# sterngerlach/my-lidar-graph-slam-v2

Hardware: AMD Instinct MI355X
Metric: candidate poses scored/sec (CSM+BnB), 1/2/4/8 GPU; % HBM roofline (higher is better)
Workload: dtype f32+u32; 1 GPU; configs[1]: frontend CSM, 1080-beam scan, 400x400@5cm grid, +-2 m/+-30 deg window at 5 cm/0.5 deg, L=4; distinct_scans=512, mode=csm_score_windows_dev, 256 windows per launch chain, 12 chains per step, beams=1080, parallelism=single GPU, poses_found=3072

## Files before the change

### include/csm_hip.h

```cpp
#ifndef CSM_HIP_H
#define CSM_HIP_H

#include <stdint.h>

#ifdef __cplusplus
extern "C" {
#endif

#define CSM_OK       0
#define CSM_ENOENT  (-2)
#define CSM_EIO     (-5)
#define CSM_ENOMEM  (-12)
#define CSM_ENODEV  (-19)
#define CSM_EINVAL  (-22)

#define CSM_FLAG_EDGE_BAND   1u
#define CSM_FLAG_KEY_TIE     2u
#define CSM_FLAG_F64_TIE     4u
#define CSM_FLAG_LITERAL     8u
#define CSM_FLAG_PROJ_DELTA 16u

typedef struct csm_ctx csm_ctx;

#define CSM_TUNE_NO_LANE_MAP         1u
#define CSM_TUNE_NO_XCD_MAP          2u
#define CSM_TUNE_NO_PAIR_TAIL        4u
#define CSM_TUNE_NO_TWO_SLICES       8u
#define CSM_TUNE_NO_THETA_MAJOR     16u
#define CSM_TUNE_NO_TILE_SPLIT      32u
#define CSM_TUNE_MAP_HOST_PROJECTION 64u
#define CSM_TUNE_NO_JOINT          128u
#define CSM_TUNE_NO_BOUND_PASS     256u
#define CSM_TUNE_NO_TWO_PHASE      512u
#define CSM_TUNE_FORCE_TWO_PHASE  1024u
#define CSM_TUNE_NO_GRAPHS        2048u

typedef struct {
    int32_t  device_id;
    uint32_t tuning_off;
    int32_t  map_uncertain_cap;
    int32_t  reserved[5];
} csm_config;

typedef struct {
    double  resolution;
    double  offset_x;
    double  offset_y;
} csm_geometry;

typedef struct {
// ... 114 lines not shown
int  csm_score_windows_dump_dev(csm_ctx* ctx, int32_t n, const uint64_t* map_ids,
                                const csm_window* windows, const int32_t* const* hit_col_dev,
                                const int32_t* const* hit_row_dev, csm_result* out_dev,
                                uint32_t* const* dump_s_dev, uint16_t* const* dump_k_dev,
                                float* const* dump_f_dev);
typedef struct {
    int64_t nominal_candidates;
    int64_t coarse_nodes_scored;
    int64_t fine_candidates_scored;
    int32_t two_phase;
    int32_t graph_replayed;
    int64_t blocks_scored, blocks_skipped;
} csm_search_info;
int  csm_last_search_info(csm_ctx* ctx, csm_search_info* out);
int  csm_bound_pass_stats(csm_ctx* ctx, uint64_t* blocks_scored, uint64_t* blocks_skipped);
int  csm_resolve_window_dev(csm_ctx* ctx, uint64_t map_id, const csm_window* w,
                            const int32_t* hit_col_dev, const int32_t* hit_row_dev,
                            csm_result* out_dev);
int  csm_score_window_dump(csm_ctx* ctx, uint64_t map_id, const csm_window* w,
                           const int32_t* hit_col, const int32_t* hit_row,
                           csm_result* out, uint32_t* dump_s, uint16_t* dump_k,
                           uint16_t* dump_coarse_k);

int  csm_correlative_match(csm_ctx* ctx, uint64_t map_id,
                           const csm_geometry* geom, const csm_scan* scan,
                           const double initial_pose[3],
                           const csm_correlative_params* params,
                           csm_summary* out);

int  csm_bnb_match_batch(csm_ctx* ctx, const csm_loop_query* queries,
// ... 515 lines not shown
                     const double* query_travel, int32_t n_q, const csm_loop_search_params* params,
                     csm_loop_candidate* out, int32_t* counts, csm_loop_search_info* info);
int  csm_host_loop_candidates_nearest(const csm_loop_candidate* cands, const int32_t* counts, int32_t n_q,
                                      int32_t n_per_query, int32_t n_total, csm_loop_candidate* out,
                                      int32_t* n_out);

int  csm_enable_kernel_timing(csm_ctx* ctx, int32_t enable);
int  csm_kernel_time(csm_ctx* ctx, const char* name, double* total_ms,
                     int64_t* launches);
int  csm_reset_kernel_timing(csm_ctx* ctx);

const char* csm_version(void);

int  csm_debug_live_bytes(int64_t* device, int64_t* pinned);
int  csm_debug_grid_known(csm_ctx* ctx, uint64_t map_id, int32_t out[2]);

#ifdef __cplusplus
}
#endif
#endif
```

### my-lidar-graph-slam-v2_amd/csm_hip/_lib.py

```python
import ctypes as C
import importlib.util
import os
import sys

_HERE = os.path.dirname(os.path.abspath(__file__))
LIB_PATH = os.environ.get("CSM_HIP_LIB") or os.path.join(os.path.dirname(_HERE), "csrc", "libcsm_hip.so")

CSM_OK = 0
CSM_ENOENT = -2
CSM_EIO = -5
CSM_ENOMEM = -12
CSM_ENODEV = -19
CSM_EINVAL = -22

FLAG_EDGE_BAND = 1
FLAG_KEY_TIE = 2
FLAG_F64_TIE = 4
FLAG_LITERAL = 8
FLAG_PROJ_DELTA = 16


class Config(C.Structure):
    _fields_ = [("device_id", C.c_int32), ("tuning_off", C.c_uint32), ("map_uncertain_cap", C.c_int32),
                ("reserved", C.c_int32 * 5)]


TUNE_NO_LANE_MAP, TUNE_NO_XCD_MAP, TUNE_NO_PAIR_TAIL, TUNE_NO_TWO_SLICES = 1, 2, 4, 8
TUNE_NO_THETA_MAJOR, TUNE_NO_TILE_SPLIT, TUNE_MAP_HOST_PROJECTION, TUNE_NO_JOINT = 16, 32, 64, 128
TUNE_NO_BOUND_PASS = 256
TUNE_NO_TWO_PHASE, TUNE_FORCE_TWO_PHASE, TUNE_NO_GRAPHS = 512, 1024, 2048
TUNE_GREEDY_LITERAL_SUMS = 4096
GREEDY_KERNEL_SIZE_MAX = 8
GROUP_FORCE_RCCL = 1


class SearchInfo(C.Structure):
    _fields_ = [("nominal_candidates", C.c_int64), ("coarse_nodes_scored", C.c_int64),
                ("fine_candidates_scored", C.c_int64), ("two_phase", C.c_int32), ("graph_replayed", C.c_int32),
                ("blocks_scored", C.c_int64), ("blocks_skipped", C.c_int64)]


class Geometry(C.Structure):
    _fields_ = [("resolution", C.c_double), ("offset_x", C.c_double),
                ("offset_y", C.c_double)]


# ... 312 lines not shown
                                   C.c_void_p, C.c_void_p, C.c_int32, C.c_void_p,
                                   C.c_void_p, C.c_void_p, C.c_void_p]),
    "csm_host_probability_lut": (None, [C.c_void_p]),
    "csm_project_scan": (C.c_int, [_ctx, _P(Geometry), C.c_void_p, C.c_double, C.c_int32, C.c_void_p,
                                   C.c_void_p, C.c_int32, C.c_void_p, C.c_void_p, C.c_void_p, C.c_int32,
                                   _P(C.c_int32)]),
    "csm_score_window": (C.c_int, [_ctx, C.c_uint64, _P(Window), C.c_void_p,
                                   C.c_void_p, _P(Result)]),
    "csm_score_window_dev": (C.c_int, [_ctx, C.c_uint64, _P(Window), C.c_void_p,
                                       C.c_void_p, C.c_void_p]),
    "csm_score_windows_dev": (C.c_int, [_ctx, C.c_int32, C.c_void_p, C.c_void_p, C.c_void_p, C.c_void_p,
                                        C.c_void_p]),
    "csm_score_windows_dump_dev": (C.c_int, [_ctx, C.c_int32, C.c_void_p, C.c_void_p, C.c_void_p, C.c_void_p,
                                             C.c_void_p, C.c_void_p, C.c_void_p, C.c_void_p]),
    "csm_bound_pass_stats": (C.c_int, [_ctx, _P(C.c_uint64), _P(C.c_uint64)]),
    "csm_last_search_info": (C.c_int, [_ctx, C.c_void_p]),
    "csm_resolve_window_dev": (C.c_int, [_ctx, C.c_uint64, _P(Window), C.c_void_p,
                                         C.c_void_p, C.c_void_p]),
    "csm_score_window_dump": (C.c_int, [_ctx, C.c_uint64, _P(Window), C.c_void_p,
                                        C.c_void_p, _P(Result), C.c_void_p,
                                        C.c_void_p, C.c_void_p]),
    "csm_correlative_match": (C.c_int, [_ctx, C.c_uint64, _P(Geometry), _P(Scan),
                                        C.c_void_p, _P(CorrelativeParams), _P(Summary)]),
    "csm_score_window_peaks": (C.c_int, [_ctx, C.c_uint64, _P(Window), C.c_void_p, C.c_void_p, _P(PeaksParams),
                                         _P(Result), _P(C.c_int32)]),
    "csm_correlative_peaks": (C.c_int, [_ctx, C.c_uint64, _P(Geometry), _P(Scan), C.c_void_p,
                                        _P(CorrelativeParams), _P(PeaksParams), _P(Summary), _P(C.c_int32)]),
    "csm_correlative_peaks_batch": (C.c_int, [_ctx, _P(LoopQuery), C.c_int32, _P(CorrelativeParams),
                                              _P(PeaksParams), _P(Summary), _P(C.c_int32)]),
    "csm_score_window_moments": (C.c_int, [_ctx, C.c_uint64, _P(Window), C.c_void_p, C.c_void_p, _P(VolumeParams),
# ... 95 lines not shown
    "csm_group_size": (C.c_int32, [C.c_void_p]),
    "csm_group_member": (C.c_void_p, [C.c_void_p, C.c_int32]),
    "csm_group_last_error": (C.c_char_p, [C.c_void_p]),
    "csm_group_bnb_match_batch": (C.c_int, [C.c_void_p, _P(LoopQuery), C.c_int32, _P(BnbParams), _P(Summary)]),
    "csm_group_correlative_match_batch": (C.c_int, [C.c_void_p, _P(LoopQuery), C.c_int32,
                                                    _P(CorrelativeParams), _P(Summary)]),
    "csm_allgather_results": (C.c_int, [C.c_void_p, C.c_void_p]),
    "csm_group_gathered_records_dev": (C.c_int, [C.c_void_p, C.c_int32, _P(C.c_void_p), _P(C.c_int32)]),
    "csm_group_exchange_info": (C.c_int, [C.c_void_p, _P(C.c_int32), _P(C.c_double)]),
    "csm_enable_kernel_timing": (C.c_int, [_ctx, C.c_int32]),
    "csm_kernel_time": (C.c_int, [_ctx, C.c_char_p, _P(C.c_double), _P(C.c_int64)]),
    "csm_reset_kernel_timing": (C.c_int, [_ctx]),
    "csm_version": (C.c_char_p, []),
    "csm_debug_live_bytes": (C.c_int, [_P(C.c_int64), _P(C.c_int64)]),
    "csm_debug_grid_known": (C.c_int, [_ctx, C.c_uint64, _P(C.c_int32)]),
}

_lib = None


def load():
    global _lib
    if _lib is not None:
        return _lib
    if not os.path.exists(LIB_PATH):
        raise ImportError(
            "libcsm_hip.so not built: run `python -c 'import __graft_entry__ as g; g.build()'` "
            "(expected at %s)" % LIB_PATH)
    if "torch" not in sys.modules and importlib.util.find_spec("torch") is not None:
        import torch
# ... 8 lines not shown
```

### my-lidar-graph-slam-v2_amd/csm_hip/api.py

```python
import contextlib
import ctypes as C

import numpy as np

from . import _lib as L


class CsmError(RuntimeError):
    def __init__(self, code, text):
        super().__init__("csm_hip error %d: %s" % (code, text))
        self.code = code


def _ptr(a):
    return a.ctypes.data_as(C.c_void_p)


def _f64(a):
    return np.ascontiguousarray(a, dtype=np.float64)


def _scan_nodes(nodes, as_f64, keep):
    arr = (L.ScanNode * max(len(nodes), 1))()
    for i, nd in enumerate(nodes):
# ... 691 lines not shown
            raise ValueError("upload_grid_blocks: every block must be (%d, %d)" % (side, side))
        ptrs = (C.c_void_p * len(keep))(*[None if b is None else b.ctypes.data for b in keep])
        self._check(self.lib.csm_upload_grid_blocks(self._ctx, map_id, ptrs, block_rows, block_cols, log2_block))
        self.shapes[map_id] = (block_rows << log2_block, block_cols << log2_block)

    def has_grid(self, map_id):
        return bool(self.lib.csm_has_grid(self._ctx, map_id))

    def debug_grid_known(self, map_id):
        out = (C.c_int32 * 2)()
        rc = self.lib.csm_debug_grid_known(self._ctx, map_id, out)
        if rc != 0:
            raise CsmError(rc, "csm_debug_grid_known: map %d not resident" % map_id)
        return out[0], out[1]

    def release_grid(self, map_id):
        self._check(self.lib.csm_release_grid(self._ctx, map_id))
        self.shapes.pop(map_id, None)

    def build_pyramid(self, map_id, win_sizes):
        w = np.ascontiguousarray(win_sizes, dtype=np.int32)
        self._check(self.lib.csm_build_pyramid(
            self._ctx, map_id, w.ctypes.data_as(C.POINTER(C.c_int32)), w.size))

    def project_scan(self, geom, sensor_pose, step_theta, win_theta, angles, ranges, cap=1 << 20):
        a, r = _f64(angles), _f64(ranges)
        n, nt = a.size, 2 * win_theta + 1
        col = np.zeros((nt, n), np.int32)
        row = np.zeros((nt, n), np.int32)
        unc = np.zeros(cap, np.uint32)
# ... 86 lines not shown
        n, ids, wins, cols, rows = prepared

        def arr(ptrs):
            return (C.c_void_p * n)(*[p or None for p in ptrs]) if ptrs is not None else None
        self._check(self.lib.csm_score_windows_dump_dev(self._ctx, n, ids, wins, cols, rows, C.c_void_p(out_ptr),
                                                        arr(dump_s_ptrs), arr(dump_k_ptrs), arr(dump_f_ptrs)))

    def last_search_info(self):
        info = L.SearchInfo()
        self._check(self.lib.csm_last_search_info(self._ctx, C.byref(info)))
        return {k: getattr(info, k) for k, _ in info._fields_}

    def bound_pass_stats(self):
        a, b = C.c_uint64(0), C.c_uint64(0)
        self._check(self.lib.csm_bound_pass_stats(self._ctx, C.byref(a), C.byref(b)))
        return a.value, b.value

    def correlative_match(self, map_id, geom, angles, ranges, rel_pose, init_pose,
                          range_x, range_y, range_theta, low_resolution,
                          score_threshold=0.0, known_rate_threshold=0.0):
        scan, keep = _scan_struct(angles, ranges, rel_pose)
        g = L.Geometry(*geom)
        p = _correlative_params(range_x, range_y, range_theta, low_resolution, score_threshold, known_rate_threshold)
        init = _f64(init_pose)
        out = L.Summary()
        self._check(self.lib.csm_correlative_match(self._ctx, map_id, C.byref(g), C.byref(scan),
                                                   _ptr(init), C.byref(p), C.byref(out)))
        return summary_to_dict(out)

    @staticmethod
# ... 671 lines not shown
```

### my-lidar-graph-slam-v2_amd/csrc/csm_api.hip

```cpp
#include "csm_matchers.hpp"
#include "csm_certify.hpp"

namespace csm_host {

void base_changed(DeviceGrid& g)
{
    g.phase.clear();
    ++g.base_epoch;
}

void free_levels(DeviceGrid& g, bool keep_base)
{
    base_changed(g);
    if (!keep_base) {
        g.xg.reset();
        g.xgf.reset();
        g.alloc.reset();
        g.xg_stale = true;
        g.xgf_valid = false;
        g.alloc_log2 = kDefaultLog2Block;
        g.alloc_derived = true;
        g.alloc_stale = true;
    }
    g.levels.resize(keep_base && !g.levels.empty() ? 1 : 0);
// ... 38 lines not shown
        return CSM_ENODEV;
    const int dev = cfg ? cfg->device_id : 0;
    if (dev < 0 || dev >= ndev)
        return CSM_ENODEV;
    csm_ctx* ctx = new csm_ctx();
    ctx->device = dev;
    {
        Tuning& t = ctx->tune;
        const uint32_t off = cfg ? cfg->tuning_off : 0u;
        t.lane_map = !(off & CSM_TUNE_NO_LANE_MAP);
        t.xcd_map = !(off & CSM_TUNE_NO_XCD_MAP);
        t.pair_tail = !(off & CSM_TUNE_NO_PAIR_TAIL);
        t.two_slices = !(off & CSM_TUNE_NO_TWO_SLICES);
        t.joint = !(off & CSM_TUNE_NO_JOINT);
        t.bound_pass = !(off & CSM_TUNE_NO_BOUND_PASS);
        t.two_phase = (off & CSM_TUNE_NO_TWO_PHASE) ? -1 : (off & CSM_TUNE_FORCE_TWO_PHASE) ? 1 : 0;
        t.graphs = !(off & CSM_TUNE_NO_GRAPHS);
        t.tile_split = !(off & CSM_TUNE_NO_TILE_SPLIT);
        t.map_host_projection = (off & CSM_TUNE_MAP_HOST_PROJECTION) != 0;
        t.greedy_literal = (off & CSM_TUNE_GREEDY_LITERAL_SUMS) != 0;
        if (off & CSM_TUNE_NO_THETA_MAJOR)
            t.theta_major = 0;
        t.map_unc_cap = cfg ? cfg->map_uncertain_cap : 0;
#ifdef CSM_TUNING
        auto env_int = [](const char* name, int dflt) {
            const char* e = getenv(name);
            return e ? atoi(e) : dflt;
        };
        t.lane_map = env_int("CSM_LANE_MAP", t.lane_map) != 0;
        t.xcd_map = env_int("CSM_XCD_MAP", t.xcd_map) != 0;
// ... 454 lines not shown
```

### my-lidar-graph-slam-v2_amd/csrc/csm_batch.hip

```cpp
#include "csm_matchers.hpp"

#include <optional>

#ifdef CSM_BIN_TIMING
static unsigned long long* g_bin_debug = nullptr;
static uint32_t* bin_debug_buffer()
{
    const size_t bytes = (size_t)kBinDebugRows * 128;
    if (!g_bin_debug && (hipMalloc(reinterpret_cast<void**>(&g_bin_debug), bytes) != hipSuccess ||
                         hipMemset(g_bin_debug, 0, bytes) != hipSuccess))
        g_bin_debug = nullptr;
    return reinterpret_cast<uint32_t*>(g_bin_debug);
}
#endif

namespace csm_host {


struct BatchPrep : WindowFrame {
    DeviceGrid* grid = nullptr;
    int level[kMaxElig] = { 0 };
    int n_theta = 0, n = 0;
    int win_x = 0, win_y = 0, win_t = 0;
    int max_tiles = 0;
// ... 420 lines not shown
    F = score_job(gr, gr.levels[p.level[0]].cells, 1, B, min_known);
    F.joint = joint ? 1 : 0;
    F.rank_l = spec.bnb ? 1 : spec.unit;
    for (int h = 1; h <= H; ++h) {
        B.band_win[h - 1] = spec.stride[h];
        B.band_nx[h - 1] = p.nx / spec.stride[h];
        B.band_ny[h - 1] = p.ny / spec.stride[h];
        ScoreJob& S = sj[h][k];
        S = score_job(gr, gr.levels[p.level[h]].cells, spec.stride[h], B, min_known);
        S.joint = F.joint;
        S.rank_l = F.rank_l;
        S.skip_unless_band = spec.bnb ? 1 : (min_known <= 1 && !coarse_first);
        S.sorted_pb = B.sorted_rc;
        S.acc_s = lvl_s + p.lvl_off[h];
        S.acc_k = lvl_k + p.lvl_off[h];
        F.elig[h - 1] = EligLevel { S.acc_k, S.acc_s, S.stride, S.nx, S.ny };
        ZeroJob& Z0 = zj[(size_t)k * H + (h - 1)];
        Z0 = ZeroJob { S.acc_s, S.acc_k, coarse_first ? 0 : (size_t)p.n_theta * S.nx * S.ny, flags,
                       S.skip_unless_band ? 0 : 1, 0 };
        zero_words_max = std::max(zero_words_max, Z0.words);
    }
    F.xg = gr.xg.as<uint32_t>();
    F.xg_pitch = gr.xg_pitch;
    F.xg_pad = gr.xg_pad;
    F.block_best = ctx->b_best.as<BlockBest>() + p.best_off;
    if (bound_pass) {
        if (!coarse_first)
            F.xgf = gr.xgf.as<float>();
        F.approx_best = ctx->b_abest.as<float>() + p.best_off;
        F.approx_slack = 4.0f * (float)(p.n + 3) * 5.9604645e-08f;
// ... 17 lines not shown
    FinalJob& Z = fj[k];
    Z = final_job(F, p.n_theta * lp[0].ncb(), I.hit_col, I.hit_row, score_thr(k), ctx->lut_dev.as<double>(),
                  resident ? resident->out_dev + i : d_out + k);
    if (spec.bnb) {
        Z.init_x = Z.init_y = Z.init_theta = 0;
    }
}

int BatchGroup::fill_job_tables()
{
    ij.resize(nq);
    bj.resize(nq);
    fj.resize(nq);
    sj.assign(H + 1, std::vector<ScoreJob>(nq));
    zj.resize((size_t)nq * H);
    for (int k = 0; k < nq; ++k)
        build_jobs(k);
    return CSM_OK;
}


static int take_pinned(csm_ctx* ctx, size_t bytes, PinBuf* out)
{
    for (size_t b = 0; b < ctx->pin_free.size(); ++b)
        if (ctx->pin_free[b].cap >= bytes) {
            *out = std::move(ctx->pin_free[b]);
            ctx->pin_free.erase(ctx->pin_free.begin() + b);
            return CSM_OK;
        }
    return grow(ctx, *out, bytes, bytes + bytes / 4 + 4096, false);
// ... 48 lines not shown
    } else {
        ScopedTimer tm(ctx, "bin");
        if ((rc = launched_ok(ctx, csm_launch::bin_batch(ctx->stream, ctx->device, n_theta_max, nq, bin_lds,
                                                         reinterpret_cast<const BinJob*>(d_bj)), "binning")))
            return rc;
    }
    if (H > 0 && zero_words_max > 0) {
        const int zb = (int)std::min<size_t>(64, (zero_words_max + 255) / 256);
        if ((rc = launched_ok(ctx, csm_launch::zero_if_band_batch(ctx->stream, std::max(1, zb), nq * H,
                                                                  reinterpret_cast<const ZeroJob*>(d_zj)), "edge-band clear")))
            return rc;
    }
    for (int h = H; h >= 1; --h) {
        if (coarse_first) {
            ScopedTimer tm(ctx, "score_bound");
            if ((rc = launched_ok(ctx, csm_launch::coarse_joint_batch(ctx->stream, lp[h].nx * lp[h].ny, (n_theta_max + 1) / 2, nq,
                                                                      reinterpret_cast<const ScoreJob*>(d_sj[h])), "coarse level")))
                return rc;
            continue;
        }
        const long blocks = (long)lp[h].ncb() * n_theta_max * nq;
        bool all_exit = true;
        for (int k = 0; k < nq; ++k)
            all_exit = all_exit && sj[h][k].skip_unless_band;
        const int n_slices = (blocks >= 2048 || all_exit)
                                 ? 1 : (int)std::min<long>(8, ceil_div(2048, (int)std::max<long>(1, blocks)));
        ScopedTimer tm(ctx, "score_coarse");
        if ((rc = launch_score_batch(ctx, reinterpret_cast<const ScoreJob*>(d_sj[h]), nq, lp[h],
                                     n_theta_max, n_slices, all_exit && nq >= 16 ? 4 : 0)))
            return rc;
    }
// ... 302 lines not shown
    return CSM_OK;
}

int csm_copy_last_batch_records(csm_ctx* ctx, csm_result* dst_dev)
{
    if (!ctx || !dst_dev)
        return fail(ctx, CSM_EINVAL, "csm_copy_last_batch_records: bad arguments");
    if (ctx->rec_n < 1 || !ctx->rec_dev.p)
        return fail(ctx, CSM_ENOENT, "no batch has been scored on this context");
    HIP_TRY(ctx, hipSetDevice(ctx->device));
    HIP_TRY(ctx, hipMemcpyAsync(dst_dev, ctx->rec_dev.p, (size_t)ctx->rec_n * sizeof(csm_result),
                                hipMemcpyDeviceToDevice, ctx->stream));
    return CSM_OK;
}

int csm_bound_pass_stats(csm_ctx* ctx, uint64_t* blocks_scored, uint64_t* blocks_skipped)
{
    if (!ctx)
        return CSM_EINVAL;
    uint32_t h[2] = { 0, 0 };
    if (ctx->bound_stats.p) {
        HIP_TRY(ctx, hipSetDevice(ctx->device));
        HIP_TRY(ctx, hipMemcpyAsync(h, ctx->bound_stats.p, 8, hipMemcpyDeviceToHost, ctx->stream));
        HIP_TRY(ctx, hipMemsetAsync(ctx->bound_stats.p, 0, 8, ctx->stream));
        HIP_TRY(ctx, hipStreamSynchronize(ctx->stream));
    }
    if (blocks_scored) *blocks_scored = h[0];
    if (blocks_skipped) *blocks_skipped = h[1];
    return CSM_OK;
}
// ... 27 lines not shown
```

### my-lidar-graph-slam-v2_amd/csrc/csm_internal.hpp

```cpp
#ifndef CSM_INTERNAL_HPP
#define CSM_INTERNAL_HPP

#include <hip/hip_runtime.h>

#include <algorithm>
#include <array>
#include <chrono>
#include <limits>
#include <cmath>
#include <cstdarg>
#include <cstdio>
#include <cstdlib>
#include <cstring>
#include <map>
#include <memory>
#include <mutex>
#include <queue>
#include <string>
#include <thread>
#include <tuple>
#include <atomic>
#include <utility>
#include <vector>

// ... 96 lines not shown
    std::vector<TimedSpan> spans;
    double  total_ms = 0.0;
    int64_t launches = 0;
};

}
using namespace csm_host;

struct Tuning {
    bool lane_map = true;
    bool xcd_map = true;
    bool pair_tail = true;
    bool two_slices = true;
    bool joint = true;
    bool bound_pass = true;
    int  two_phase = 0;
    bool graphs = true;
    bool tile_split = true;
    bool map_host_projection = false;
    bool greedy_literal = false;
    int  theta_major = -1;
    int  fine_slices = 0, force_r = 0, pair_r = 0, pair_ncbx = 0, pair_groups = 0, pair_ls = 0,
         pair_tail_ls = 0, nbuf = 0, map_unc_cap = 0;
    bool plan_debug = false, host_timing = false;
};

struct csm_ctx {
    int device = 0;
    Tuning tune;
    hipStream_t own_stream = nullptr;
// ... 36 lines not shown
    DevBuf pr_tab;
    PinBuf pr_pin;
    DevBuf lf_tab;
    PinBuf lf_pin;
    DevBuf rc_tab, rc_work;
    PinBuf rc_pin, rc_back;
    DevBuf ps_tab, ps_work, ps_fix;
    PinBuf ps_pin, ps_back;
    DevBuf ls_dev;
    PinBuf ls_pin;
    DevBuf pg_buf;
    DevBuf pg_s;
    std::vector<uint8_t> pg_stage;
    DevBuf pg_cov;
    std::vector<uint8_t> pg_cov_stage;
    DevBuf rec_dev;
    int rec_n = 0;
    std::vector<csm_result> rec_patch;
    DevBuf m_rays, m_recs, m_cell, m_lists, m_cnt, m_lut;
    DevBuf m_alloc;
    double m_lut_hit = -1.0, m_lut_miss = -1.0;
    int m_cus = 0;
    DevBuf m_btab;
    std::vector<double> stage;
    std::vector<std::pair<hipEvent_t, PinBuf>> resident_hold;
    unsigned flag_toggle = 0;
    bool flags_ready = false;
    bool fine_acc_dirty = false;
    int timing = 0;
    std::map<std::string, KernelTimer> timers;
// ... 186 lines not shown
```

### my-lidar-graph-slam-v2_amd/csrc/csm_joint.hpp

```cpp
#ifndef CSM_JOINT_HPP
#define CSM_JOINT_HPP

#include "csm_launch.hpp"

namespace csm_launch {

int binj_hash_size(int n_points);
size_t binj_lds_bytes(int tiles, int n_points, int hash_size);

int binj_batch(hipStream_t s, int device, int n_pairs_max, int n_jobs, size_t lds, const BinJob* jobs);

int joint_batch(const ScoreLaunch& a, const ScoreJob* jobs);

int binj_one(hipStream_t s, int device, int n_pairs, size_t lds, const BinJob& job);
int joint_one(const ScoreLaunch& a, const ScoreJob& job, int n_pairs);

int bound_select(hipStream_t s, const ScoreJob* jobs, int n_jobs, int ncb, int split_cb, uint32_t* items0,
                 uint32_t* items1, uint32_t* counts, uint32_t cap, int round);

int coarse_joint_batch(hipStream_t s, int nodes, int n_pairs_max, int n_jobs, const ScoreJob* jobs);
int unit_bounds(hipStream_t s, const ScoreJob* jobs, int n_jobs, int units_max, int cbx, int cby, int ncbx, int ncb);

int expand_pairs_f(hipStream_t s, const uint16_t* cells, int rows, int cols, int pitch, float* xgf, int xg_prows,
                   int xg_pitch, int pad);

}
#endif
```

### my-lidar-graph-slam-v2_amd/csrc/csm_joint_kernels.hip

```cpp
#include <hip/hip_runtime.h>
#include <stdint.h>

#include <type_traits>

#include "csm_score_common.hpp"
#include "csm_joint.hpp"

namespace csm {

#ifdef CSM_BIN_TIMING
#define BINJ_TICK(k)                                                                  \
    do {                                                                              \
        if (threadIdx.x == 0 && job.tuning_counters) {                                \
            const unsigned long long now_ = __builtin_readcyclecounter();             \
            reinterpret_cast<unsigned long long*>(job.tuning_counters)[dbg_row_ * 16 + (k)] += now_ - tick_; \
            tick_ = now_;                                                             \
        }                                                                             \
    } while (0)
#else
#define BINJ_TICK(k) do { } while (0)
#endif
constexpr int kBinjNoBeam = 0x3fffffff;
constexpr int kBinjBlock = 512;

// ... 908 lines not shown
                                                                 const uint16_t* lane_map, int xcd_map, BlockBase bb)
{
    int bx, by, bz;
    xcd_block(xcd_map, bx, by, bz);
    score_body_joint<LS, R>(jobs[bz], cbx, groups, lane_map, bx, by, bb);
}

template <int LS, int R>
__global__ __launch_bounds__(kBlock, 4) void k_score_joint_one(ScoreJob job, int cbx, int groups,
                                                               const uint16_t* lane_map, int n_pairs, BlockBase bb)
{
    const int by = (int)(blockIdx.x % (uint32_t)n_pairs), bx = (int)(blockIdx.x / (uint32_t)n_pairs);
    score_body_joint<LS, R>(job, cbx, groups, lane_map, bx, by, bb);
}

__global__ __launch_bounds__(256) void k_coarse_joint_batch(const ScoreJob* jobs)
{
    auto uni = [](int v) { return __builtin_amdgcn_readfirstlane(v); };
    const ScoreJob& job = jobs[blockIdx.z];
    const int n_theta = uni(job.n_theta);
    const int tp = (int)blockIdx.y, t0 = 2 * tp;
    const int nx = uni(job.nx), ny = uni(job.ny), nodes = nx * ny;
    const int node = (int)blockIdx.x * 256 + (int)threadIdx.x;
    if (t0 >= n_theta || uni(node) >= nodes)
        return;
    const bool two = t0 + 1 < n_theta;
    const bool on = node < nodes;
    const int nd = on ? node : 0;
    const int yi = nd / nx, xi = nd - yi * nx;
    const int stride = uni(job.stride), pitch = uni(job.pitch), rows = uni(job.rows), cols = uni(job.cols);
    const int dx = xi * stride, dy = yi * stride;
    const uint32_t lane_off = (uint32_t)(dy * pitch + dx);
    const int x_lo = uni(job.x_lo), y_lo = uni(job.y_lo);
    const uint16_t* __restrict__ cells = job.cells;
    const int ntiles = uni(job.n_tiles[tp]);
    const TileRec* __restrict__ recs = job.tiles + (size_t)tp * job.max_tiles;
    const uint32_t* __restrict__ pbs = job.sorted_pb + (size_t)tp * 2 * job.n_points;

    uint32_t S0 = 0, S1 = 0, KK = 0;
    auto add = [&](uint32_t v, uint32_t m0, uint32_t m1) {
        S0 = mad_u24(v, m0, S0);
        S1 = mad_u24(v, m1, S1);
        KK = mad_u24(min(v, 1u), m0 | (m1 << 16), KK);
    };
    const int lane = (int)threadIdx.x & 63;
    auto rl = [](uint32_t v, int l) { return (uint32_t)__builtin_amdgcn_readlane((int)v, l); };
    auto rec_group = [&](int ti) {
        const int i = ti * 8 + lane;
        return i < ntiles * 8 ? reinterpret_cast<const uint32_t*>(recs)[i] : 0u;
    };
    auto entries = [&](uint32_t first, int n) { return lane < n ? pbs[first + lane] : 0u; };
    uint32_t recw = ntiles > 0 ? rec_group(0) : 0u;
    uint32_t ent_nxt = ntiles > 0 ? entries(rl(recw, 2), (int)rl(recw, 3)) : 0u;
    for (int ti = 0; ti < ntiles; ++ti) {
// ... 50 lines not shown
                    const bool c_ok = c >= 0 && c < cols;
                    if (e & 0x0f0f0000u) {
                        const bool ok = c_ok && r >= 0 && r < rows;
                        const uint32_t v = cells[ok ? (size_t)r * pitch + c : 0];
                        add(ok ? v : 0u, (e >> 16) & 15u, (e >> 24) & 15u);
                    }
                    if (e & 0xf0f00000u) {
                        const bool ok = c_ok && r + 1 >= 0 && r + 1 < rows;
                        const uint32_t v = cells[ok ? (size_t)(r + 1) * pitch + c : 0];
                        add(ok ? v : 0u, (e >> 20) & 15u, e >> 28);
                    }
                }
            }
        }
    }
    if (!on)
        return;
    const size_t per_slice = (size_t)nodes;
    const size_t ai = (size_t)t0 * per_slice + (size_t)xi * ny + yi;
    job.acc_s[ai] = S0;
    job.acc_k[ai] = KK & 0xffffu;
    if (two) {
        job.acc_s[ai + per_slice] = S1;
        job.acc_k[ai + per_slice] = KK >> 16;
    }
}

__global__ __launch_bounds__(256) void k_unit_bounds(const ScoreJob* jobs, int cbx, int cby, int ncbx, int ncb)
{
    const ScoreJob& job = jobs[blockIdx.y];
    const int unit = (int)blockIdx.x * 4 + (int)(threadIdx.x >> 6);
    const int lane = (int)threadIdx.x & 63;
    if (unit >= job.n_theta * ncb || !job.approx_best || job.n_elig < 1)
        return;
    const int t = unit / ncb, cb = unit - t * ncb;
    const int by = cb / ncbx, bx = cb - by * ncbx;
    const EligLevel& el = job.elig[0];
    const int L = el.div;
    const int xc0 = bx * cbx / L, xc1 = (min(job.nx, (bx + 1) * cbx) - 1) / L;
    const int yc0 = by * cby / L, yc1 = (min(job.ny, (by + 1) * cby) - 1) / L;
// ... 154 lines not shown

int joint_one(const ScoreLaunch& a, const ScoreJob& job, int n_pairs)
{
    return match_pair_shape(a, [&](auto ls, auto r) {
        return launch_lds(a.device, k_score_joint_one<ls, r>, dim3((unsigned)n_pairs * a.grid.x), dim3(kBlock), a.lds,
                          a.stream, job, a.cbx, a.groups, a.lane_map, n_pairs, a.bb);
    });
}

int bound_select(hipStream_t s, const ScoreJob* jobs, int n_jobs, int ncb, int split_cb, uint32_t* items0,
                 uint32_t* items1, uint32_t* counts, uint32_t cap, int round)
{
    return launch(k_bound_select, dim3(n_jobs), dim3(256), s, jobs, ncb, split_cb, items0, items1, counts, cap, round);
}

int coarse_joint_batch(hipStream_t s, int nodes, int n_pairs_max, int n_jobs, const ScoreJob* jobs)
{
    return launch(k_coarse_joint_batch, dim3((nodes + 255) / 256, n_pairs_max, n_jobs), dim3(256), s, jobs);
}

int unit_bounds(hipStream_t s, const ScoreJob* jobs, int n_jobs, int units_max, int cbx, int cby, int ncbx, int ncb)
{
    return launch(k_unit_bounds, dim3((units_max + 3) / 4, n_jobs), dim3(256), s, jobs, cbx, cby, ncbx, ncb);
}

int expand_pairs_f(hipStream_t s, const uint16_t* cells, int rows, int cols, int pitch, float* xgf, int xg_prows,
                   int xg_pitch, int pad)
{
    const size_t total = (size_t)xg_prows * xg_pitch;
    const int blocks = (int)(total + 255 < 4096 * 256 ? (total + 255) / 256 : 4096);
    return launch(k_expand_pairs_f, dim3(blocks), dim3(256), s, cells, rows, cols, pitch,
                  reinterpret_cast<float2*>(xgf), xg_prows, xg_pitch, pad);
}
// ... 3 lines not shown
```

Before: 60.05 billion candidate poses/s.

## Stage coarse-level grid windows in LDS and batch theta pairs per workgroup

Adds a new coarse-level bound kernel. Each workgroup covers a chunk of node rows, stages the needed subsampled map window for each column phase into 64 KiB of LDS, and builds per-phase item lists. It then accumulates scores for up to eight theta pairs from that shared image instead of making direct global reads per node. When the LDS budget does not fit, it falls back to smaller pair groups or to the old direct path. The change also adds stats counters and debug entry points, and it brings more syncs, atomics and LDS occupancy pressure.

```diff
diff --git a/include/csm_hip.h b/include/csm_hip.h
--- a/include/csm_hip.h
+++ b/include/csm_hip.h
@@ -34,6 +34,7 @@
 #define CSM_TUNE_NO_TWO_PHASE      512u
 #define CSM_TUNE_FORCE_TWO_PHASE  1024u
 #define CSM_TUNE_NO_GRAPHS        2048u
+#define CSM_TUNE_NO_LEVEL_LDS     8192u
 
 typedef struct {
     int32_t  device_id;
@@ -178,6 +179,7 @@
 } csm_search_info;
 int  csm_last_search_info(csm_ctx* ctx, csm_search_info* out);
 int  csm_bound_pass_stats(csm_ctx* ctx, uint64_t* blocks_scored, uint64_t* blocks_skipped);
+int  csm_level_path_stats(csm_ctx* ctx, uint64_t* lds_workgroups, uint64_t* direct_workgroups);
 int  csm_resolve_window_dev(csm_ctx* ctx, uint64_t map_id, const csm_window* w,
                             const int32_t* hit_col_dev, const int32_t* hit_row_dev,
                             csm_result* out_dev);
@@ -723,6 +725,8 @@
 
 int  csm_debug_live_bytes(int64_t* device, int64_t* pinned);
 int  csm_debug_grid_known(csm_ctx* ctx, uint64_t map_id, int32_t out[2]);
+int  csm_debug_level_sums(csm_ctx* ctx, int32_t k, uint32_t* out_s, uint32_t* out_k, size_t cap, int32_t dims[3]);
+int  csm_debug_set_level_pairs(csm_ctx* ctx, int32_t pairs);
 
 #ifdef __cplusplus
 }
diff --git a/my-lidar-graph-slam-v2_amd/csm_hip/_lib.py b/my-lidar-graph-slam-v2_amd/csm_hip/_lib.py
--- a/my-lidar-graph-slam-v2_amd/csm_hip/_lib.py
+++ b/my-lidar-graph-slam-v2_amd/csm_hip/_lib.py
@@ -30,6 +30,7 @@
 TUNE_NO_BOUND_PASS = 256
 TUNE_NO_TWO_PHASE, TUNE_FORCE_TWO_PHASE, TUNE_NO_GRAPHS = 512, 1024, 2048
 TUNE_GREEDY_LITERAL_SUMS = 4096
+TUNE_NO_LEVEL_LDS = 8192
 GREEDY_KERNEL_SIZE_MAX = 8
 GROUP_FORCE_RCCL = 1
 
@@ -372,6 +373,7 @@
     "csm_score_windows_dump_dev": (C.c_int, [_ctx, C.c_int32, C.c_void_p, C.c_void_p, C.c_void_p, C.c_void_p,
                                              C.c_void_p, C.c_void_p, C.c_void_p, C.c_void_p]),
     "csm_bound_pass_stats": (C.c_int, [_ctx, _P(C.c_uint64), _P(C.c_uint64)]),
+    "csm_level_path_stats": (C.c_int, [_ctx, _P(C.c_uint64), _P(C.c_uint64)]),
     "csm_last_search_info": (C.c_int, [_ctx, C.c_void_p]),
     "csm_resolve_window_dev": (C.c_int, [_ctx, C.c_uint64, _P(Window), C.c_void_p,
                                          C.c_void_p, C.c_void_p]),
@@ -497,6 +499,8 @@
     "csm_version": (C.c_char_p, []),
     "csm_debug_live_bytes": (C.c_int, [_P(C.c_int64), _P(C.c_int64)]),
     "csm_debug_grid_known": (C.c_int, [_ctx, C.c_uint64, _P(C.c_int32)]),
+    "csm_debug_set_level_pairs": (C.c_int, [_ctx, C.c_int32]),
+    "csm_debug_level_sums": (C.c_int, [_ctx, C.c_int32, _P(C.c_uint32), _P(C.c_uint32), C.c_size_t, _P(C.c_int32)]),
 }
 
 _lib = None
diff --git a/my-lidar-graph-slam-v2_amd/csm_hip/api.py b/my-lidar-graph-slam-v2_amd/csm_hip/api.py
--- a/my-lidar-graph-slam-v2_amd/csm_hip/api.py
+++ b/my-lidar-graph-slam-v2_amd/csm_hip/api.py
@@ -729,6 +729,20 @@
             raise CsmError(rc, "csm_debug_grid_known: map %d not resident" % map_id)
         return out[0], out[1]
 
+    def debug_set_level_pairs(self, pairs):
+        self._check(self.lib.csm_debug_set_level_pairs(self._ctx, pairs))
+
+    def debug_level_sums(self, k):
+        dims = (C.c_int32 * 3)()
+        rc = self.lib.csm_debug_level_sums(self._ctx, k, None, None, 0, dims)
+        if rc != 0:
+            raise CsmError(rc, "csm_debug_level_sums: no level sums of window %d" % k)
+        shape = (dims[0], dims[1], dims[2])
+        s, kn = np.zeros(shape, np.uint32), np.zeros(shape, np.uint32)
+        self._check(self.lib.csm_debug_level_sums(self._ctx, k, s.ctypes.data_as(C.POINTER(C.c_uint32)),
+                                                  kn.ctypes.data_as(C.POINTER(C.c_uint32)), s.size, dims))
+        return s, kn
+
     def release_grid(self, map_id):
         self._check(self.lib.csm_release_grid(self._ctx, map_id))
         self.shapes.pop(map_id, None)
@@ -845,6 +859,11 @@
     def bound_pass_stats(self):
         a, b = C.c_uint64(0), C.c_uint64(0)
         self._check(self.lib.csm_bound_pass_stats(self._ctx, C.byref(a), C.byref(b)))
+        return a.value, b.value
+
+    def level_path_stats(self):
+        a, b = C.c_uint64(0), C.c_uint64(0)
+        self._check(self.lib.csm_level_path_stats(self._ctx, C.byref(a), C.byref(b)))
         return a.value, b.value
 
     def correlative_match(self, map_id, geom, angles, ranges, rel_pose, init_pose,
diff --git a/my-lidar-graph-slam-v2_amd/csrc/csm_api.hip b/my-lidar-graph-slam-v2_amd/csrc/csm_api.hip
--- a/my-lidar-graph-slam-v2_amd/csrc/csm_api.hip
+++ b/my-lidar-graph-slam-v2_amd/csrc/csm_api.hip
@@ -76,6 +76,7 @@
         t.two_slices = !(off & CSM_TUNE_NO_TWO_SLICES);
         t.joint = !(off & CSM_TUNE_NO_JOINT);
         t.bound_pass = !(off & CSM_TUNE_NO_BOUND_PASS);
+        t.level_lds = !(off & CSM_TUNE_NO_LEVEL_LDS);
         t.two_phase = (off & CSM_TUNE_NO_TWO_PHASE) ? -1 : (off & CSM_TUNE_FORCE_TWO_PHASE) ? 1 : 0;
         t.graphs = !(off & CSM_TUNE_NO_GRAPHS);
         t.tile_split = !(off & CSM_TUNE_NO_TILE_SPLIT);
diff --git a/my-lidar-graph-slam-v2_amd/csrc/csm_batch.hip b/my-lidar-graph-slam-v2_amd/csrc/csm_batch.hip
--- a/my-lidar-graph-slam-v2_amd/csrc/csm_batch.hip
+++ b/my-lidar-graph-slam-v2_amd/csrc/csm_batch.hip
@@ -458,6 +458,11 @@
         S.sorted_pb = B.sorted_rc;
         S.acc_s = lvl_s + p.lvl_off[h];
         S.acc_k = lvl_k + p.lvl_off[h];
+        if (coarse_first) {
+            S.bound_stats = ctx->bound_stats.as<uint32_t>();
+            if (h == H)
+                ctx->last_level_sums.push_back({ idx[k], p.lvl_off[h], lvl_total + p.lvl_off[h], p.n_theta, S.nx, S.ny });
+        }
         F.elig[h - 1] = EligLevel { S.acc_k, S.acc_s, S.stride, S.nx, S.ny };
         ZeroJob& Z0 = zj[(size_t)k * H + (h - 1)];
         Z0 = ZeroJob { S.acc_s, S.acc_k, coarse_first ? 0 : (size_t)p.n_theta * S.nx * S.ny, flags,
@@ -505,6 +510,7 @@
     fj.resize(nq);
     sj.assign(H + 1, std::vector<ScoreJob>(nq));
     zj.resize((size_t)nq * H);
+    ctx->last_level_sums.clear();
     for (int k = 0; k < nq; ++k)
         build_jobs(k);
     return CSM_OK;
@@ -583,7 +589,8 @@
     for (int h = H; h >= 1; --h) {
         if (coarse_first) {
             ScopedTimer tm(ctx, "score_bound");
-            if ((rc = launched_ok(ctx, csm_launch::coarse_joint_batch(ctx->stream, lp[h].nx * lp[h].ny, (n_theta_max + 1) / 2, nq,
+            if ((rc = launched_ok(ctx, csm_launch::coarse_joint_batch(ctx->stream, ctx->device, ctx->tune.level_lds, ctx->tune.level_pairs, lp[h].nx,
+                                                                      lp[h].ny, (n_theta_max + 1) / 2, nq,
                                                                       reinterpret_cast<const ScoreJob*>(d_sj[h])), "coarse level")))
                 return rc;
             continue;
@@ -916,6 +923,59 @@
     return CSM_OK;
 }
 
+int csm_level_path_stats(csm_ctx* ctx, uint64_t* lds_workgroups, uint64_t* direct_workgroups)
+{
+    if (!ctx)
+        return CSM_EINVAL;
+    uint32_t h[2] = { 0, 0 };
+    if (ctx->bound_stats.p) {
+        char* const at = reinterpret_cast<char*>(ctx->bound_stats.p) + 8;
+        HIP_TRY(ctx, hipSetDevice(ctx->device));
+        HIP_TRY(ctx, hipMemcpyAsync(h, at, 8, hipMemcpyDeviceToHost, ctx->stream));
+        HIP_TRY(ctx, hipMemsetAsync(at, 0, 8, ctx->stream));
+        HIP_TRY(ctx, hipStreamSynchronize(ctx->stream));
+    }
+    if (lds_workgroups) *lds_workgroups = h[0];
+    if (direct_workgroups) *direct_workgroups = h[1];
+    return CSM_OK;
+}
+
+int csm_debug_set_level_pairs(csm_ctx* ctx, int32_t pairs)
+{
+    if (!ctx || !(pairs == 0 || pairs == 1 || pairs == 2 || pairs == 4 || pairs == 8))
+        return CSM_EINVAL;
+    ctx->tune.level_pairs = pairs;
+    return CSM_OK;
+}
+
+int csm_debug_level_sums(csm_ctx* ctx, int32_t k, uint32_t* out_s, uint32_t* out_k, size_t cap, int32_t dims[3])
+{
+    if (!ctx || !dims)
+        return CSM_EINVAL;
+    const csm_ctx::LevelSums* w = nullptr;
+    for (const csm_ctx::LevelSums& e : ctx->last_level_sums)
+        if (e.query == k)
+            w = &e;
+    if (!w || !ctx->b_lvl.p)
+        return CSM_ENOENT;
+    dims[0] = w->n_theta;
+    dims[1] = w->nxc;
+    dims[2] = w->nyc;
+    const size_t words = (size_t)w->n_theta * w->nxc * w->nyc;
+    if (!out_s && !out_k)
+        return CSM_OK;
+    if (cap < words)
+        return CSM_EINVAL;
+    const uint32_t* lvl = ctx->b_lvl.as<uint32_t>();
+    HIP_TRY(ctx, hipSetDevice(ctx->device));
+    if (out_s)
+        HIP_TRY(ctx, hipMemcpyAsync(out_s, lvl + w->s_off, words * 4, hipMemcpyDeviceToHost, ctx->stream));
+    if (out_k)
+        HIP_TRY(ctx, hipMemcpyAsync(out_k, lvl + w->k_off, words * 4, hipMemcpyDeviceToHost, ctx->stream));
+    HIP_TRY(ctx, hipStreamSynchronize(ctx->stream));
+    return CSM_OK;
+}
+
 int csm_bound_pass_stats(csm_ctx* ctx, uint64_t* blocks_scored, uint64_t* blocks_skipped)
 {
     if (!ctx)
diff --git a/my-lidar-graph-slam-v2_amd/csrc/csm_internal.hpp b/my-lidar-graph-slam-v2_amd/csrc/csm_internal.hpp
--- a/my-lidar-graph-slam-v2_amd/csrc/csm_internal.hpp
+++ b/my-lidar-graph-slam-v2_amd/csrc/csm_internal.hpp
@@ -134,6 +134,8 @@
     bool two_slices = true;
     bool joint = true;
     bool bound_pass = true;
+    bool level_lds = true;
+    int  level_pairs = 0;
     int  two_phase = 0;
     bool graphs = true;
     bool tile_split = true;
@@ -200,6 +202,12 @@
     std::vector<uint8_t> pg_stage;
     DevBuf pg_cov;
     std::vector<uint8_t> pg_cov_stage;
+    struct LevelSums {
+        int query;
+        size_t s_off, k_off;
+        int n_theta, nxc, nyc;
+    };
+    std::vector<LevelSums> last_level_sums;
     DevBuf rec_dev;
     int rec_n = 0;
     std::vector<csm_result> rec_patch;
diff --git a/my-lidar-graph-slam-v2_amd/csrc/csm_joint.hpp b/my-lidar-graph-slam-v2_amd/csrc/csm_joint.hpp
--- a/my-lidar-graph-slam-v2_amd/csrc/csm_joint.hpp
+++ b/my-lidar-graph-slam-v2_amd/csrc/csm_joint.hpp
@@ -18,7 +18,8 @@
 int bound_select(hipStream_t s, const ScoreJob* jobs, int n_jobs, int ncb, int split_cb, uint32_t* items0,
                  uint32_t* items1, uint32_t* counts, uint32_t cap, int round);
 
-int coarse_joint_batch(hipStream_t s, int nodes, int n_pairs_max, int n_jobs, const ScoreJob* jobs);
+int coarse_joint_batch(hipStream_t s, int device, bool level_lds, int force_pairs, int nx, int ny, int n_pairs_max,
+                       int n_jobs, const ScoreJob* jobs);
 int unit_bounds(hipStream_t s, const ScoreJob* jobs, int n_jobs, int units_max, int cbx, int cby, int ncbx, int ncb);
 
 int expand_pairs_f(hipStream_t s, const uint16_t* cells, int rows, int cols, int pitch, float* xgf, int xg_prows,
diff --git a/my-lidar-graph-slam-v2_amd/csrc/csm_joint_kernels.hip b/my-lidar-graph-slam-v2_amd/csrc/csm_joint_kernels.hip
--- a/my-lidar-graph-slam-v2_amd/csrc/csm_joint_kernels.hip
+++ b/my-lidar-graph-slam-v2_amd/csrc/csm_joint_kernels.hip
@@ -1,6 +1,8 @@
 #include <hip/hip_runtime.h>
+#include <limits.h>
 #include <stdint.h>
 
+#include <algorithm>
 #include <type_traits>
 
 #include "csm_score_common.hpp"
@@ -946,22 +948,11 @@
     score_body_joint<LS, R>(job, cbx, groups, lane_map, bx, by, bb);
 }
 
-__global__ __launch_bounds__(256) void k_coarse_joint_batch(const ScoreJob* jobs)
+__device__ __forceinline__ void coarse_pair_direct(const ScoreJob& job, int tp, int dx, int dy, uint32_t& S0,
+                                                   uint32_t& S1, uint32_t& KK)
 {
     auto uni = [](int v) { return __builtin_amdgcn_readfirstlane(v); };
-    const ScoreJob& job = jobs[blockIdx.z];
-    const int n_theta = uni(job.n_theta);
-    const int tp = (int)blockIdx.y, t0 = 2 * tp;
-    const int nx = uni(job.nx), ny = uni(job.ny), nodes = nx * ny;
-    const int node = (int)blockIdx.x * 256 + (int)threadIdx.x;
-    if (t0 >= n_theta || uni(node) >= nodes)
-        return;
-    const bool two = t0 + 1 < n_theta;
-    const bool on = node < nodes;
-    const int nd = on ? node : 0;
-    const int yi = nd / nx, xi = nd - yi * nx;
-    const int stride = uni(job.stride), pitch = uni(job.pitch), rows = uni(job.rows), cols = uni(job.cols);
-    const int dx = xi * stride, dy = yi * stride;
+    const int pitch = uni(job.pitch), rows = uni(job.rows), cols = uni(job.cols);
     const uint32_t lane_off = (uint32_t)(dy * pitch + dx);
     const int x_lo = uni(job.x_lo), y_lo = uni(job.y_lo);
     const uint16_t* __restrict__ cells = job.cells;
@@ -969,7 +960,7 @@
     const TileRec* __restrict__ recs = job.tiles + (size_t)tp * job.max_tiles;
     const uint32_t* __restrict__ pbs = job.sorted_pb + (size_t)tp * 2 * job.n_points;
 
-    uint32_t S0 = 0, S1 = 0, KK = 0;
+    S0 = S1 = KK = 0;
     auto add = [&](uint32_t v, uint32_t m0, uint32_t m1) {
         S0 = mad_u24(v, m0, S0);
         S1 = mad_u24(v, m1, S1);
@@ -1050,6 +1041,25 @@
             }
         }
     }
+}
+
+__global__ __launch_bounds__(256) void k_coarse_joint_batch(const ScoreJob* jobs)
+{
+    auto uni = [](int v) { return __builtin_amdgcn_readfirstlane(v); };
+    const ScoreJob& job = jobs[blockIdx.z];
+    const int n_theta = uni(job.n_theta);
+    const int tp = (int)blockIdx.y, t0 = 2 * tp;
+    const int nx = uni(job.nx), ny = uni(job.ny), nodes = nx * ny;
+    const int node = (int)blockIdx.x * 256 + (int)threadIdx.x;
+    if (t0 >= n_theta || uni(node) >= nodes)
+        return;
+    const bool two = t0 + 1 < n_theta;
+    const bool on = node < nodes;
+    const int nd = on ? node : 0;
+    const int yi = nd / nx, xi = nd - yi * nx;
+    const int stride = uni(job.stride);
+    uint32_t S0, S1, KK;
+    coarse_pair_direct(job, tp, xi * stride, yi * stride, S0, S1, KK);
     if (!on)
         return;
     const size_t per_slice = (size_t)nodes;
@@ -1060,6 +1070,302 @@
         job.acc_s[ai + per_slice] = S1;
         job.acc_k[ai + per_slice] = KK >> 16;
     }
+}
+
+constexpr int kLevelBlock = 512;
+constexpr int kLevelMaxL = 16;
+constexpr int kLevelLdsBytes = 64 * 1024;
+static_assert(kLevelLdsBytes / 2 <= 65536, "an item holds a 16-bit element offset");
+
+template <int P>
+__device__ __forceinline__ bool level_group(const ScoreJob& job, int tp0, int rows_per_chunk, int lds_bytes,
+                                            uint32_t* sm_level, int* s_box, uint32_t* s_cnt, uint32_t* s_off)
+{
+    auto uni = [](int v) { return __builtin_amdgcn_readfirstlane(v); };
+    const int n_theta = uni(job.n_theta);
+    const int tid = (int)threadIdx.x, lane = tid & 63, nthr = (int)blockDim.x;
+    const int nx = uni(job.nx), ny = uni(job.ny);
+    const int L = uni(job.stride);
+    const int row_base = (int)blockIdx.x * rows_per_chunk;
+    const int crows = min(rows_per_chunk, ny - row_base);
+    const bool on = tid < crows * nx;
+    const int nd = on ? tid : 0;
+    const int yl = nd / nx, xi = nd - yl * nx, yi = row_base + yl;
+    const int x_lo = uni(job.x_lo), y_lo = uni(job.y_lo);
+    const int pitch = uni(job.pitch), rows = uni(job.rows), cols = uni(job.cols);
+    const uint16_t* __restrict__ cells = job.cells;
+
+    int ntl[P], ent_n[P];
+    const TileRec* __restrict__ recs[P];
+    const uint32_t* __restrict__ pbs[P];
+#pragma unroll
+    for (int q = 0; q < P; ++q) {
+        const int tp = tp0 + q;
+        const bool live = 2 * tp < n_theta;
+        ntl[q] = live ? uni(job.n_tiles[live ? tp : tp0]) : 0;
+        recs[q] = job.tiles + (size_t)(live ? tp : tp0) * job.max_tiles;
+        pbs[q] = job.sorted_pb + (size_t)(live ? tp : tp0) * 2 * job.n_points;
+        ent_n[q] = 0;
+        if (ntl[q] > 0)
+            ent_n[q] = uni((int)(recs[q][ntl[q] - 1].start + recs[q][ntl[q] - 1].count));
+    }
+
+    int rbase[P], n_recs = 0;
+#pragma unroll
+    for (int q = 0; q < P; ++q) {
+        rbase[q] = n_recs;
+        n_recs += ntl[q];
+    }
+    const bool l_ok = L <= kLevelMaxL && (long)n_recs * 12 <= (long)lds_bytes;
+    uint32_t* const rtab = sm_level + ((lds_bytes >> 2) - (l_ok ? 3 * n_recs : 0));
+
+    if (tid < 4)
+        s_box[tid] = tid < 2 ? INT_MAX : INT_MIN;
+    for (int i = tid; i < kLevelMaxL * P; i += nthr)
+        s_cnt[i] = 0u;
+    __syncthreads();
+    {
+        int b0 = INT_MAX, b1 = INT_MAX, b2 = INT_MIN, b3 = INT_MIN;
+#pragma unroll
+        for (int q = 0; q < P; ++q)
+            for (int i = tid; i < ntl[q]; i += nthr) {
+                const TileRec r = recs[q][i];
+                b0 = min(b0, r.r0);
+                b1 = min(b1, r.c0);
+                b2 = max(b2, r.r0 + r.h);
+                b3 = max(b3, r.c0 + r.w);
+                if (l_ok) {
+                    uint32_t* const t = rtab + 3 * (rbase[q] + i);
+                    t[0] = r.start;
+                    t[1] = (uint32_t)r.r0;
+                    t[2] = (uint32_t)r.c0;
+                }
+            }
+        if (b0 != INT_MAX) {
+            atomicMin(&s_box[0], b0);
+            atomicMin(&s_box[1], b1);
+            atomicMax(&s_box[2], b2);
+            atomicMax(&s_box[3], b3);
+        }
+    }
+    __syncthreads();
+    const bool any_rec = uni(s_box[0]) != INT_MAX;
+    const int R0 = any_rec ? uni(s_box[0]) : 0, C0 = any_rec ? uni(s_box[1]) : 0;
+    const int hbox = any_rec ? uni(s_box[2]) - R0 : 1, wbox = any_rec ? uni(s_box[3]) - C0 : 1;
+    const int Rb = R0 + y_lo + L * row_base, Cb = C0 + x_lo;
+    const int himg = hbox + L * (crows - 1);
+    const int wimg = (wbox - 1) / L + nx;
+    int pimg = (wimg + 1) & ~1;
+    {
+        const int need = (nx + 1) / 2 + 1;
+        if (2 * need <= 32)
+            for (int k = 0; k < 32; ++k) {
+                const int sh = ((L * pimg) >> 1) & 31;
+                if (sh >= need && sh <= 32 - need)
+                    break;
+                pimg += 2;
+            }
+    }
+
+    auto items_of = [&](int q, int e, uint32_t w, int& ph, uint32_t& it_even, uint32_t& it_odd) {
+        const uint32_t* const t = rtab + 3 * rbase[q];
+        int lo = 0, hi = ntl[q] - 1;
+        while (lo < hi) {
+            const int mid = (lo + hi + 1) >> 1;
+            if ((int)t[3 * mid] <= e)
+                lo = mid;
+            else
+                hi = mid - 1;
+        }
+        const int dr = (int)t[3 * lo + 1] - R0 + (int)((w >> 7) & 127u);
+        const int dc = (int)t[3 * lo + 2] - C0 + (int)(w & 127u);
+        const int jc = dc / L;
+        ph = dc - jc * L;
+        const uint32_t at = (uint32_t)(dr * pimg + jc);
+        it_even = (w & 0x0f0f0000u) ? (at | ((w >> 16) & 15u) << 16 | ((w >> 24) & 15u) << 20) : 0u;
+        it_odd = (w & 0xf0f00000u) ? ((at + (uint32_t)pimg) | ((w >> 20) & 15u) << 16 | (w >> 28) << 20) : 0u;
+    };
+    auto for_entries = [&](auto&& f) {
+#pragma unroll
+        for (int q = 0; q < P; ++q)
+            for (int e0 = tid; e0 < ent_n[q]; e0 += 4 * nthr) {
+                uint32_t w[4];
+#pragma unroll
+                for (int u = 0; u < 4; ++u)
+                    w[u] = e0 + u * nthr < ent_n[q] ? pbs[q][e0 + u * nthr] : 0u;
+#pragma unroll
+                for (int u = 0; u < 4; ++u) {
+                    if (!(w[u] >> 16))
+                        continue;
+                    int ph;
+                    uint32_t ie, io;
+                    items_of(q, e0 + u * nthr, w[u], ph, ie, io);
+                    f(ph * P + q, ie, io);
+                }
+            }
+    };
+    if (l_ok)
+        for_entries([&](int slot, uint32_t ie, uint32_t io) {
+            atomicAdd(&s_cnt[slot], (ie ? 1u : 0u) + (io ? 1u : 0u));
+        });
+    __syncthreads();
+    if (tid < 64) {
+        const int lp = l_ok ? L * P : 0;
+        const int c0 = lane < lp ? (int)s_cnt[lane] : 0, c1 = lane + 64 < lp ? (int)s_cnt[lane + 64] : 0;
+        const int p0 = wave_prefix_sum(c0);
+        const int t0 = __builtin_amdgcn_readlane(p0, 63);
+        const int p1 = wave_prefix_sum(c1) + t0;
+        if (lane < lp) {
+            s_off[lane] = (uint32_t)(p0 - c0);
+            s_cnt[lane] = (uint32_t)(p0 - c0);
+        }
+        if (lane + 64 < lp) {
+            s_off[lane + 64] = (uint32_t)(p1 - c1);
+            s_cnt[lane + 64] = (uint32_t)(p1 - c1);
+        }
+        if (lane == 63)
+            s_off[lp] = (uint32_t)p1;
+    }
+    __syncthreads();
+    const int n_items = l_ok ? uni((int)s_off[L * P]) : 0;
+    const long img_elems = (long)himg * pimg;
+    const bool use_lds = l_ok && img_elems <= 65536 && (long)n_items * 4 + img_elems * 2 <= (long)lds_bytes &&
+                         (long)n_items * 4 + (long)n_recs * 12 <= (long)lds_bytes;
+    if (P > 1 && !use_lds && l_ok)
+        return false;
+
+    uint32_t S0[P], S1[P], KK[P];
+#pragma unroll
+    for (int q = 0; q < P; ++q)
+        S0[q] = S1[q] = KK[q] = 0u;
+
+    if (!use_lds) {
+#pragma unroll
+        for (int q = 0; q < P; ++q)
+            if (2 * (tp0 + q) < n_theta)
+                coarse_pair_direct(job, tp0 + q, xi * L, yi * L, S0[q], S1[q], KK[q]);
+    } else {
+        uint32_t* const list = sm_level;
+        uint16_t* const img = reinterpret_cast<uint16_t*>(sm_level + n_items);
+        for_entries([&](int slot, uint32_t ie, uint32_t io) {
+            uint32_t pos = atomicAdd(&s_cnt[slot], (ie ? 1u : 0u) + (io ? 1u : 0u));
+            if (ie)
+                list[pos++] = ie;
+            if (io)
+                list[pos] = io;
+        });
+        __syncthreads();
+        const uint16_t* const mine = img + (L * yl * pimg + xi);
+        auto rl = [](uint32_t v, int l) { return (uint32_t)__builtin_amdgcn_readlane((int)v, l); };
+        const int si0 = tid / wimg, sj0 = tid - si0 * wimg;
+        const int sdi = nthr / wimg, sdj = nthr - sdi * wimg;
+        for (int pc = 0; pc < (n_items ? L : 0); ++pc) {
+            {
+                int i = si0, j = sj0;
+                const int cbase = Cb + pc;
+                while (i < himg) {
+                    int at[8];
+                    uint16_t v[8];
+                    bool ok[8];
+#pragma unroll
+                    for (int u = 0; u < 8; ++u) {
+                        const int r = Rb + i, c = cbase + L * j;
+                        at[u] = i < himg ? i * pimg + j : -1;
+                        ok[u] = i < himg && r >= 0 && r < rows && c >= 0 && c < cols;
+                        v[u] = cells[ok[u] ? (size_t)r * pitch + c : 0];
+                        i += sdi;
+                        j += sdj;
+                        if (j >= wimg) {
+                            j -= wimg;
+                            ++i;
+                        }
+                    }
+#pragma unroll
+                    for (int u = 0; u < 8; ++u)
+                        if (at[u] >= 0)
+                            img[at[u]] = ok[u] ? v[u] : (uint16_t)0;
+                }
+            }
+            __syncthreads();
+#pragma unroll
+            for (int q = 0; q < P; ++q) {
+                const int beg = uni((int)s_off[pc * P + q]), end = uni((int)s_off[pc * P + q + 1]);
+                uint32_t nxt = beg + lane < end ? list[beg + lane] : 0u;
+                for (int j0 = beg; j0 < end; j0 += 64) {
+                    const uint32_t itm = nxt;
+                    const int m = min(64, end - j0);
+                    if (j0 + 64 < end)
+                        nxt = j0 + 64 + lane < end ? list[j0 + 64 + lane] : 0u;
+                    for (int j = 0; j < m; j += 8) {
+                        uint32_t w[8], v[8];
+#pragma unroll
+                        for (int u = 0; u < 8; ++u) {
+                            w[u] = rl(itm, j + u);
+                            v[u] = mine[w[u] & 0xffffu];
+                        }
+#pragma unroll
+                        for (int u = 0; u < 8; ++u) {
+                            uint32_t m0, m1, mk, known;
+                            asm("s_bfe_u32 %0, %3, 0x40010\n\t"
+                                "s_bfe_u32 %1, %3, 0x40014\n\t"
+                                "s_lshl_b32 %2, %1, 16\n\t"
+                                "s_or_b32 %2, %2, %0"
+                                : "=&s"(m0), "=&s"(m1), "=&s"(mk)
+                                : "s"(w[u])
+                                : "scc");
+                            asm("v_min_u32 %0, 1, %1" : "=v"(known) : "v"(v[u]));
+                            S0[q] = mad_u24(v[u], m0, S0[q]);
+                            S1[q] = mad_u24(v[u], m1, S1[q]);
+                            KK[q] = mad_u24(known, mk, KK[q]);
+                        }
+                    }
+                }
+            }
+            __syncthreads();
+        }
+    }
+    if (tid == 0 && job.bound_stats)
+        atomicAdd(job.bound_stats + (use_lds ? 2 : 3), 1u);
+    const size_t per_slice = (size_t)nx * ny;
+#pragma unroll
+    for (int q = 0; q < P; ++q) {
+        const int t0 = 2 * (tp0 + q);
+        if (t0 >= n_theta || !on)
+            continue;
+        const size_t ai = (size_t)t0 * per_slice + (size_t)xi * ny + yi;
+        job.acc_s[ai] = S0[q];
+        job.acc_k[ai] = KK[q] & 0xffffu;
+        if (t0 + 1 < n_theta) {
+            job.acc_s[ai + per_slice] = S1[q];
+            job.acc_k[ai + per_slice] = KK[q] >> 16;
+        }
+    }
+    return true;
+}
+
+template <int P>
+__device__ __forceinline__ void level_run(const ScoreJob& job, int tp0, int rows_per_chunk, int lds_bytes,
+                                          uint32_t* sm_level, int* s_box, uint32_t* s_cnt, uint32_t* s_off)
+{
+    if (2 * tp0 >= __builtin_amdgcn_readfirstlane(job.n_theta))
+        return;
+    if (level_group<P>(job, tp0, rows_per_chunk, lds_bytes, sm_level, s_box, s_cnt, s_off))
+        return;
+    if constexpr (P > 1) {
+#pragma unroll 1
+        for (int h = 0; h < 2; ++h)
+            level_run<P / 2>(job, tp0 + h * (P / 2), rows_per_chunk, lds_bytes, sm_level, s_box, s_cnt, s_off);
+    }
+}
+
+template <int P>
+__global__ __launch_bounds__(kLevelBlock) void k_level_lds_batch(const ScoreJob* jobs, int rows_per_chunk, int lds_bytes)
+{
+    extern __shared__ __attribute__((aligned(16))) uint32_t sm_level[];
+    __shared__ int s_box[4];
+    __shared__ uint32_t s_cnt[kLevelMaxL * P];
+    __shared__ uint32_t s_off[kLevelMaxL * P + 1];
+    level_run<P>(jobs[blockIdx.z], (int)blockIdx.y * P, rows_per_chunk, lds_bytes, sm_level, s_box, s_cnt, s_off);
 }
 
 __global__ __launch_bounds__(256) void k_unit_bounds(const ScoreJob* jobs, int cbx, int cby, int ncbx, int ncb)
@@ -1244,9 +1550,30 @@
     return launch(k_bound_select, dim3(n_jobs), dim3(256), s, jobs, ncb, split_cb, items0, items1, counts, cap, round);
 }
 
-int coarse_joint_batch(hipStream_t s, int nodes, int n_pairs_max, int n_jobs, const ScoreJob* jobs)
-{
-    return launch(k_coarse_joint_batch, dim3((nodes + 255) / 256, n_pairs_max, n_jobs), dim3(256), s, jobs);
+int coarse_joint_batch(hipStream_t s, int device, bool level_lds, int force_pairs, int nx, int ny, int n_pairs_max,
+                       int n_jobs, const ScoreJob* jobs)
+{
+    const int nodes = nx * ny;
+    if (!level_lds || nx > kLevelBlock)
+        return launch(k_coarse_joint_batch, dim3((nodes + 255) / 256, n_pairs_max, n_jobs), dim3(256), s, jobs);
+    const int rows_per_chunk = nodes <= kLevelBlock ? ny : kLevelBlock / nx;
+    const int chunks = (ny + rows_per_chunk - 1) / rows_per_chunk;
+    const int block = (std::min(ny, rows_per_chunk) * nx + 63) / 64 * 64;
+    int p = 1;
+    for (int c : { 8, 4, 2 })
+        if (n_jobs > 1 && (long)chunks * ((n_pairs_max + c - 1) / c) * n_jobs >= 4096) {
+            p = c;
+            break;
+        }
+    if (force_pairs == 1 || force_pairs == 2 || force_pairs == 4 || force_pairs == 8)
+        p = force_pairs;
+    const dim3 grid(chunks, (n_pairs_max + p - 1) / p, n_jobs);
+    switch (p) {
+    case 8: return launch_lds(device, k_level_lds_batch<8>, grid, dim3(block), kLevelLdsBytes, s, jobs, rows_per_chunk, kLevelLdsBytes);
+    case 4: return launch_lds(device, k_level_lds_batch<4>, grid, dim3(block), kLevelLdsBytes, s, jobs, rows_per_chunk, kLevelLdsBytes);
+    case 2: return launch_lds(device, k_level_lds_batch<2>, grid, dim3(block), kLevelLdsBytes, s, jobs, rows_per_chunk, kLevelLdsBytes);
+    default: return launch_lds(device, k_level_lds_batch<1>, grid, dim3(block), kLevelLdsBytes, s, jobs, rows_per_chunk, kLevelLdsBytes);
+    }
 }
 
 int unit_bounds(hipStream_t s, const ScoreJob* jobs, int n_jobs, int units_max, int cbx, int cby, int ncbx, int ncb)
```

Measured after the change: 84.78 billion candidate poses/s, median of 6. +41.2%, better.
